# LeonOrou/OPF-Graph-Neural-Solver

Measured on AMD Instinct MI355X. Metric: grids/sec (fwd+bwd) on batched case118, K=4, higher is better.
Workload: dtype f32

## Files before the change

opf-graph-neural-solver_amd/csrc/gns_api.hip:

```cpp
#include <atomic>
#include <cmath>
#include <cstring>
#include <cstdlib>
#include <mutex>
#include <vector>
#include "gns_kernels.h"
#include "gns_gridwg.h"

namespace {
struct GnsTuning {
  int fwd_mapping;
  int gw_pack;
  int fwd_waves;
  int fwd_plane;
  int dw_mfma;
  int train_mapping;
  int bwd_variant;
  int team;
  int bwds_mode;
  int bwds_chunks;
  int bwds_save;
};

bool waves_ok(int& w) { return w > 0 && (w & (w - 1)) == 0 && w * 64 <= GNS_FWD_MAX_THREADS; }
bool chunks_ok(int& c) { return c == 0 || gns_part_index(c) >= 0; }
bool as_flag(int& v) { v = v ? 1 : 0; return true; }
int env_int(const char* e) { return std::atoi(e); }
int env_mapping(const char* e) { return !std::strcmp(e, "lane") ? 1 : (!std::strcmp(e, "lds") ? 2 : 0); }
int env_plane(const char* e) { return e[0] == '0' ? 0 : (e[0] == '1' ? 1 : 2); }
int env_flag(const char* e) { return e[0] == '0' ? 0 : 1; }
struct GnsOption {
  const char* name; int GnsTuning::*member; int lo, hi; bool (*check)(int&); const char* env; int (*parse)(const char*);
  bool accepts(int& v) const { return check ? check(v) : (v >= lo && v <= hi); }
};
const GnsOption g_options[] = {
  {"fwd_mapping",   &GnsTuning::fwd_mapping,   0, 2,            nullptr,   "GNS_FWD_MAPPING",   env_mapping},
  {"train_mapping", &GnsTuning::train_mapping, 0, 2,            nullptr,   "GNS_TRAIN_MAPPING", env_mapping},
  {"bwd_variant",   &GnsTuning::bwd_variant,   1, 4,            nullptr,   "GNS_BWD_VARIANT",   env_int},
  {"gw_pack",       &GnsTuning::gw_pack,       0, 16,           nullptr,   "GNS_GW_PACK",       env_int},
  {"fwd_waves",     &GnsTuning::fwd_waves,     0, 0,            waves_ok,  "GNS_FWD_WAVES",     env_int},
  {"fwd_plane",     &GnsTuning::fwd_plane,     0, 2,            nullptr,   "GNS_FWD_PLANE",     env_plane},
  {"dw_mfma",       &GnsTuning::dw_mfma,       0, 0,            as_flag,   "GNS_DW_MFMA",       env_flag},
  {"team",          &GnsTuning::team,          0, GNS_MAX_TEAM, nullptr,   "GNS_TEAM",          env_int},
  {"bwds_mode",     &GnsTuning::bwds_mode,     0, 2,            nullptr,   "GNS_BWDS_MODE",     env_int},
  {"bwds_chunks",   &GnsTuning::bwds_chunks,   0, 0,            chunks_ok, "GNS_BWDS_CHUNKS",   env_int},
  {"bwds_save",     &GnsTuning::bwds_save,     0, 1,            nullptr,   "GNS_BWDS_SAVE",     env_int},
};
GnsTuning make_tuning() {
  GnsTuning t{0, 0, GNS_FWD_THREADS / 64, 2, 1, 0, 4, 0, 1, 0, 1};
  for (const GnsOption& o : g_options)
    if (const char* e = std::getenv(o.env)) { int v = o.parse(e); if (o.accepts(v)) t.*o.member = v; }
  return t;
}
GnsTuning& tuning() {
  static GnsTuning t = make_tuning();
  return t;
}

struct GnsLast {
  int fwd_kernel, fwd_waves, fwd_plane, team, gw_pack;
  int bwd_kernel, dw_mfma, bwds_mode, bwds_chunks, bwds_R, bwd_gw_pack;
  int bwds_save;
};
GnsLast g_last{-1, -1, -1, -1, -1, -1, -1, -1, -1, -1, -1, -1};
struct GnsLastName { const char* name; int GnsLast::*member; };
const GnsLastName g_last_names[] = {
  {"fwd_kernel", &GnsLast::fwd_kernel}, {"fwd_waves", &GnsLast::fwd_waves}, {"fwd_plane", &GnsLast::fwd_plane}, {"team", &GnsLast::team},
  {"gw_pack", &GnsLast::gw_pack}, {"bwd_kernel", &GnsLast::bwd_kernel}, {"dw_mfma", &GnsLast::dw_mfma}, {"bwds_mode", &GnsLast::bwds_mode},
  {"bwds_chunks", &GnsLast::bwds_chunks}, {"bwds_R", &GnsLast::bwds_R}, {"bwd_gw_pack", &GnsLast::bwd_gw_pack},
  {"bwds_save", &GnsLast::bwds_save},
};
void record_forward(int kernel, int waves, int plane, int team, int pack) {
  g_last.fwd_kernel = kernel; g_last.fwd_waves = waves; g_last.fwd_plane = plane; g_last.team = team; g_last.gw_pack = pack;
}
void record_backward(int kernel, int dw_mfma, int mode, int chunks, int R, int pack, int save = 0) {
  g_last.bwd_kernel = kernel; g_last.dw_mfma = dw_mfma; g_last.bwds_mode = mode; g_last.bwds_chunks = chunks; g_last.bwds_R = R;
  g_last.bwd_gw_pack = pack; g_last.bwds_save = save;
}

constexpr int GNS_MAX_DEVICES = 64;
struct GnsDevice {
  int ncu;
  int gw_ready;
  int split_ready;
  int fwd_ready;
};
const GnsDevice& device() {
  static GnsDevice devs[GNS_MAX_DEVICES];
  static std::atomic<int> done[GNS_MAX_DEVICES];
  static std::mutex mu;
  static const GnsDevice none{0, 0, 0, 0};
  int dev = 0;
// ... 239 lines not shown
int lane_forward(const gns_config* cfg, const GnsFamilies& fam, const GnsFwdLayout& L, char* ws, float* pt, float* pin,
                 const int* topo_dev, const int* group_topo, const int* slot_grid, int64_t Bt, float* v, float* theta,
                 float* total_loss, float* last_loss, int save_state, hipStream_t st) {
  const int N = cfg->n_bus, E = cfg->n_line, K = cfg->K, d = cfg->latent_dim, h = cfg->hidden_dim;
  const GnsTuning& T = tuning();
  int rc;
  GnsFwdArgs A;
  std::memset(&A, 0, sizeof(A));
  A.topo = topo_dev; A.group_topo = group_topo; A.slot_grid = slot_grid; A.pt = pt; A.in = pin;
  A.state = (float*)(ws + L.off_state); A.lam = (float*)(ws + L.off_lam); A.msg = (float*)(ws + L.off_msg);
  A.v_out = v; A.theta_out = theta; A.total_out = total_loss; A.last_out = last_loss;
  fill_forward_families(A, fam);
  fill_loss_weights(A, cfg);
  A.Bt = Bt; A.G = L.groups; A.N = N; A.E = E; A.K = K; A.save = save_state ? 1 : 0;
  A.save_a1 = saves_first_layer(cfg, save_state, group_topo != nullptr) ? 1 : 0;
  const int team0 = lane_team(L.groups * GNS_LANES);
  A.team = team0;
  A.team_ws = (unsigned char*)(ws + L.off_team);
  int waves = T.fwd_waves;
  while (waves * A.team > GNS_MAXP) waves /= 2;
  A.part_idx = gns_part_index(waves * A.team);
  auto pick_planes = [&]() {
    A.plane = (device().fwd_ready && gns_fwd_plane_fits(N, A.team) && T.fwd_plane) ? 1 : 0;
    if (A.plane && gns_fwd_plane2_fits(N, A.team) && T.fwd_plane == 2) A.plane = 2;
  };
  pick_planes();
  if (A.team > 1) {
    const int per_cu = gns_fwd_blocks_per_cu(d, h, cfg->multiple_phi, A, waves * 64);
    if ((long long)per_cu * device().ncu < A.G * A.team) {
      A.team = 1;
      waves = T.fwd_waves;
      A.part_idx = gns_part_index(waves);
      pick_planes();
    }
  }
  if (team0 > 1 && hipMemsetAsync(A.team_ws, 0, (size_t)L.groups * GNS_TEAM_CTR_BYTES, st) != hipSuccess) return GNS_ELAUNCH;
  record_forward(1, waves, A.plane, A.team, -1);
  prof_mark(0, true, st);
  rc = gns_launch_forward(d, h, cfg->multiple_phi, A, waves * 64, st);
  prof_mark(0, false, st);
  return rc;
}

int split_backward(const gns_config* cfg, const GnsFamilies& fam, const GnsFwdLayout& L, const GnsBwdsLayout& S, const char* fw,
                   char* bw, const int* topo_dev, const int* group_topo, const int* slot_grid, const float* params,
                   const void* packed_inputs, int64_t Bt, const float* grad_total, const float* grad_last, const float* grad_v,
                   const float* grad_theta, float* grad_params, hipStream_t st, const IgradOut* ig = nullptr) {
  const int N = cfg->n_bus, E = cfg->n_line, K = cfg->K, d = cfg->latent_dim, h = cfg->hidden_dim;
  int rc;
  GnsBwdsArgs A;
  std::memset(&A, 0, sizeof(A));
  A.topo = topo_dev; A.group_topo = group_topo; A.slot_grid = slot_grid;
  A.pt = (const float*)(fw + L.off_pt); A.pn = (const float*)(fw + L.off_pn);
  A.in = packed_inputs ? (const float*)packed_inputs : (const float*)(fw + L.off_in);
  A.state = (const float*)(fw + L.off_state); A.lam = (const float*)(fw + L.off_lam); A.msg = (const float*)(fw + L.off_msg);
  A.g_total = grad_total; A.g_last = grad_last; A.g_v = grad_v; A.g_theta = grad_theta;
  A.adj = (float*)(bw + S.off_adj); A.slots = (float*)(bw + S.off_slots); A.slab = (float*)(bw + S.off_slab);
  fill_backward_families(A, fam);
  A.Bt = Bt; A.G = S.groups; A.slab_floats = S.slab_floats; A.N = N; A.E = E; A.K = K;
  A.C = S.C; A.part_idx = gns_part_index(S.C); A.R = S.R;
  A.RB = (int)(1 + S.mq); A.RBA = (int)S.adj_rows;
  A.mode = cfg->multiple_phi ? tuning().bwds_mode : 2;
  const size_t lds = gns_bwds_phys_lds(N, &A.use_plane);
  if (ig) {
    A.igrad = ig->buf;
    if (hipMemsetAsync(A.igrad, 0, ig->bytes, st) != hipSuccess) return GNS_ELAUNCH;
  }
  A.save_a1 = saves_first_layer(cfg, ig ? GNS_SAVE_IGRAD : 1, group_topo != nullptr) ? 1 : 0;
  record_backward(4, 1, A.mode, A.C, A.R, -1, A.save_a1);
  prof_mark(1, true, st);
  for (int k = K - 1; k >= 0; --k) {
    A.k = k;
    A.gwk = loss_weight(cfg, k);
    rc = gns_launch_bwds_phys(A, lds, st);
    if (rc != GNS_OK) return rc;
    if (ig) {
      rc = gns_launch_bwds_igrad_phys(A, st);
      if (rc != GNS_OK) return rc;
    }
    rc = gns_launch_bwds_sweep(d, h, cfg->multiple_phi, A, st);
    if (rc != GNS_OK) return rc;
  }
  if (ig && (ig->buses || ig->lines || ig->gens)) {
    rc = gns_launch_bwds_igrad_unpack(A, ig->in_buses, ig->in_lines, ig->in_gens, cfg->n_gen, ig->buses, ig->lines, ig->gens, st);
// ... 442 lines not shown
```

opf-graph-neural-solver_amd/csrc/gns_backward_split.hip:

```cpp
#include "gns_device.h"
#include "gns_kernels.h"
#include "gns_dw.h"
#include "gns_phys_device.h"

typedef int gns_i8v __attribute__((ext_vector_type(8)));
#ifndef GNS_BWDS_ONE_LAYOUT
#define GNS_BWDS_ONE_LAYOUT 0
#endif
#ifndef GNS_BWDS_WPE
#define GNS_BWDS_WPE 2
#endif
#ifndef GNS_BWDS_KEEP_SLOPES
#define GNS_BWDS_KEEP_SLOPES 1
#endif
#if GNS_BWDS_KEEP_SLOPES
#define GNS_SLOPES(sl) sl
#define GNS_SLOPE_OF(sl, layer, act, u) sl[layer][u]
#else
#define GNS_SLOPES(sl) nullptr
#define GNS_SLOPE_OF(sl, layer, act, u) dlrelu2(act[u])
#endif
#ifndef GNS_BWDS_FRESH_INPUTS
#define GNS_BWDS_FRESH_INPUTS 1
#endif
// ... 5 lines not shown
#endif
#ifndef GNS_BWDS_AH_M
#define GNS_BWDS_AH_M 5
#endif
#ifndef GNS_BWDS_AH_M0
#define GNS_BWDS_AH_M0 5
#endif
#ifndef GNS_BWDS_AH_T0
#define GNS_BWDS_AH_T0 4
#endif
#ifndef GNS_BWDS_LASTK_FOLD
#define GNS_BWDS_LASTK_FOLD 0
#endif
#define GNS_BWDS_PHYS_THREADS (GNS_BWDS_PHYS_WAVES * 64)

__global__ void __launch_bounds__(GNS_BWDS_PHYS_THREADS) gns_bwds_phys_kernel(GnsBwdsArgs A) {
  extern __shared__ __attribute__((aligned(16))) float lds[];
  constexpr int W = GNS_BWDS_PHYS_WAVES;
  const int lane = threadIdx.x & 63;
  const int wave = __builtin_amdgcn_readfirstlane(threadIdx.x >> 6);
  const int N = A.N, E = A.E, K = A.K, k = A.k;
  cip topo = (cip)A.topo;
  const long long g = blockIdx.x;
  long long b = g * GNS_LANES + lane;
  bool live = b < A.Bt;
  if (A.group_topo) {
    const int s = A.slot_grid[g * GNS_LANES + lane];
    b = s;
    live = s >= 0 && s < A.Bt;
    if (!gns_group_topo(A.topo, A.group_topo, g, N, E, topo)) return;
// ... 7 lines not shown
  const int e0 = epart[wave], e1 = epart[wave + 1];
  const bool use_plane = A.use_plane != 0, plane_dp = A.use_plane == 2;
  float* const red = lds;
  float* const pl_v = lds + W * GNS_LANES;
  float* const pl_th = pl_v + (use_plane ? N * GNS_LANES : 0);
  float* const pl_dp = pl_th + (plane_dp ? N * GNS_LANES : 0);
  const long long R = gns_in_rows(N, E);
  const float* IN = A.in;
  const long long in_base = g * R, row_ein = in_base + 3LL * N, row_eout = row_ein + 3LL * E, row_grid = row_eout + E;
  const float gt = (live && A.g_total) ? A.g_total[b] : 0.f;
  const float gl = (live && A.g_last) ? A.g_last[b] : 0.f;
  const int RB = A.RB, RBA = A.RBA;
  auto state_row = [&](int slot, int n) { return (((long long)slot * A.G + g) * N + n) * RB; };
  auto adj_row = [&](int n) { return (g * N + n) * RBA; };
  auto slot_ptr = [&](int j, int p) { return A.slots + ((g * 6 + j) * E + p) * GNS_LANES + lane; };
  const f4 gsum = *row_ptr(IN, row_grid, lane);
  const float invN = 1.0f / (float)N;
  const bool last = k == K - 1;
  const int mode = A.mode;
  const bool x2_live = mode == 2 || k + 1 < K - 1;
  const float cdp = 2.f * (gt * A.gwk + (last ? gl : 0.f)) * invN;
  const f2 lamv = reinterpret_cast<const f2*>(A.lam)[((long long)k * A.G + g) * GNS_LANES + lane];
  const int bits = (int)lamv.y;
  const bool low1 = bits & 1, low2 = bits & 2;

  float lb = 0.f;
  constexpr int PB = 4;
  for (int nb = n0; nb < n1; nb += PB) {
    f4 s1[PB], a0[PB], x0[PB], x1[PB], x2[PB], b1[PB];
#pragma unroll
// ... 58 lines not shown
        L.thc = pl_th[ic * GNS_LANES + lane]; L.thd = pl_th[id * GNS_LANES + lane];
        if (plane_dp) { L.Fb = pl_dp[t * GNS_LANES + lane]; L.Tb = pl_dp[s * GNS_LANES + lane]; }
        else { L.Fb = row_ptr(A.adj, adj_row(t), lane)->z; L.Tb = row_ptr(A.adj, adj_row(s), lane)->z; }
      } else {
        const f4 ss = *row_ptr(A.state, state_row(k + 1, s), lane), st = *row_ptr(A.state, state_row(k + 1, t), lane);
        L.vs = ss.x; L.ths = ss.y; L.vt = st.x; L.tht = st.y;
        L.tha = row_ptr(A.state, state_row(k + 1, ia), lane)->y; L.thb = row_ptr(A.state, state_row(k + 1, ib), lane)->y;
        L.thc = row_ptr(A.state, state_row(k + 1, ic), lane)->y; L.thd = row_ptr(A.state, state_row(k + 1, id), lane)->y;
        L.Fb = row_ptr(A.adj, adj_row(t), lane)->z;
        L.Tb = row_ptr(A.adj, adj_row(s), lane)->z;
      }
    };
    auto edge_adjoint = [&](int p, const EdgeIn& L) {
      const LineTrig T = line_trig<false>(L.ths, L.tht, L.tha, L.thb, L.thc, L.thd, L.e1v.w, L.o0.z);
      const LineAdj R = line_state_adjoint(T, L.vs, L.vt, L.e1v.y, L.e1v.z, L.o0.x, L.o0.y, L.Fb, L.Tb, pgbar);
      if (!L.gs) *slot_ptr(0, p) = R.dvs;
      if (!L.gt) *slot_ptr(1, p) = R.dvt;
      *slot_ptr(2, p) = R.dths;
      *slot_ptr(4, p) = R.dbar; *slot_ptr(5, p) = R.dbar2;
    };
    for (int p = e0; p < e1; p += 2) {
      EdgeIn L0, L1;
      edge_load(p, L0);
      edge_load(min(p + 1, e1 - 1), L1);
      edge_adjoint(p, L0);
      if (p + 1 < e1) edge_adjoint(p + 1, L1);
    }
  }
  __syncthreads();

  for (int n = n0; n < n1; ++n) {
    const long long ar = adj_row(n);
    const f4 a0 = *row_ptr(A.adj, ar, lane);
    float vbar = a0.x, thbar = a0.y;
    const float dpb = a0.z;
    const int p0 = in_ptr[n], p1 = in_ptr[n + 1], q0 = out_ptr[n], q1 = out_ptr[n + 1], i0 = incd_ptr[n], i1 = incd_ptr[n + 1];
    const bool gen = is_gen[n] != 0;
    {
      float ai[4], bi[4], ao[4], bo[4], ci[8];
#pragma unroll
      for (int j = 0; j < 4; ++j) { const int pp = min(p0 + j, max(p1 - 1, p0)); ai[j] = gen ? 0.f : *slot_ptr(1, min(pp, E - 1)); bi[j] = -*slot_ptr(2, min(pp, E - 1)); }
#pragma unroll
      for (int j = 0; j < 4; ++j) { const int p = q2p[min(min(q0 + j, max(q1 - 1, q0)), E - 1)]; ao[j] = gen ? 0.f : *slot_ptr(0, p); bo[j] = *slot_ptr(2, p); }
#pragma unroll
      for (int j = 0; j < 8; ++j) {
        const int code = incd[min(min(i0 + j, max(i1 - 1, i0)), 4 * E - 1)];
        const float val = *slot_ptr((code & 2) ? 5 : 4, code >> 2);
        ci[j] = (code & 1) ? -val : val;
      }
#pragma unroll
      for (int j = 0; j < 4; ++j) if (p0 + j < p1) { vbar += ai[j]; thbar += bi[j]; }
#pragma unroll
      for (int j = 0; j < 4; ++j) if (q0 + j < q1) { vbar += ao[j]; thbar += bo[j]; }
#pragma unroll
      for (int j = 0; j < 8; ++j) if (i0 + j < i1) thbar += ci[j];
    }
    for (int p = p0 + 4; p < p1; p += 4) {
      float a[4], bb[4];
#pragma unroll
      for (int j = 0; j < 4; ++j) { const int pp = min(p + j, p1 - 1); a[j] = gen ? 0.f : *slot_ptr(1, pp); bb[j] = -*slot_ptr(2, pp); }
#pragma unroll
      for (int j = 0; j < 4; ++j) if (p + j < p1) { vbar += a[j]; thbar += bb[j]; }
    }
    for (int q = q0 + 4; q < q1; q += 4) {
      float a[4], bb[4];
#pragma unroll
      for (int j = 0; j < 4; ++j) { const int p = q2p[min(q + j, q1 - 1)]; a[j] = gen ? 0.f : *slot_ptr(0, p); bb[j] = *slot_ptr(2, p); }
#pragma unroll
      for (int j = 0; j < 4; ++j) if (q + j < q1) { vbar += a[j]; thbar += bb[j]; }
    }
    for (int i = i0 + 8; i < i1; i += 8) {
      float a[8];
#pragma unroll
      for (int j = 0; j < 8; ++j) {
        const int code = incd[min(i + j, i1 - 1)];
        const float val = *slot_ptr((code & 2) ? 5 : 4, code >> 2);
        a[j] = (code & 1) ? -val : val;
      }
#pragma unroll
      for (int j = 0; j < 8; ++j) if (i + j < i1) thbar += a[j];
    }
    vbar += (pgbar - dpb) * a0.w;
    *row_ptr(A.adj, ar, lane) = f4{vbar, thbar, dpb, 0.f};
  }
}

template <int D, int H, bool MULTI>
struct BwdsShape {
  using C = GnsDims<D, H, MULTI>;
  static constexpr int LIN = C::LF_IN, XL = (LIN + 1) / 2, PIN = C::PHI_IN, SOFF = 2 + D / 2;
  static constexpr int NB1 = (2 * XL + 15) / 16, NDM = (D + 15) / 16;
// ... 692 lines not shown
int gns_launch_bwds_igrad_unpack(const GnsBwdsArgs& A, const float* buses, const float* lines, const float* gens, int Gn,
                                 float* grad_buses, float* grad_lines, float* grad_gens, hipStream_t st) {
  hipLaunchKernelGGL(gns_bwds_igrad_unpack_kernel, dim3((unsigned)A.G, (unsigned)(A.N + A.E)), dim3(64), 0, st, A, buses, lines, gens, Gn,
                     grad_buses, grad_lines, grad_gens);
  return hipGetLastError() == hipSuccess ? GNS_OK : GNS_ELAUNCH;
}

int gns_bwds_supported(int d, int h, int multi) {
  (void)multi;
#define GNS_CASE(DD, HH) if (d == DD && h == HH) return 1;
  GNS_FOR_EACH_DIMS(GNS_CASE)
#undef GNS_CASE
  return 0;
}

size_t gns_bwds_phys_lds(int N, int* use_plane) {
  const size_t red = (size_t)GNS_BWDS_PHYS_WAVES * GNS_LANES * 4;
  const size_t plane = (size_t)N * GNS_LANES * 4;
  const int level = red + 3 * plane <= (size_t)160 * 1024 ? 2 : (red + 2 * plane <= (size_t)160 * 1024 ? 1 : 0);
  if (use_plane) *use_plane = level;
  return red + (level == 2 ? 3 : (level == 1 ? 2 : 0)) * plane;
}

int gns_launch_bwds_phys(const GnsBwdsArgs& A, size_t lds, hipStream_t st) {
  hipLaunchKernelGGL(gns_bwds_phys_kernel, dim3((unsigned)A.G), dim3(GNS_BWDS_PHYS_THREADS), lds, st, A);
  return hipGetLastError() == hipSuccess ? GNS_OK : GNS_ELAUNCH;
}

int gns_launch_bwds_sweep(int d, int h, int multi, const GnsBwdsArgs& A, hipStream_t st) {
  const long long GB = (A.G + A.R - 1) / A.R;
  const unsigned blocks = (unsigned)(GB * A.C);
  const bool fold_m = GNS_BWDS_LASTK_FOLD && A.k == A.K - 1 && !A.group_topo && !A.igrad;
#define GNS_SWEEP1(DD, HH, MM, FAMS, GR, IG) do { if (A.k == 0) hipLaunchKernelGGL((gns_bwds_sweep_kernel<DD, HH, MM, FAMS, true, GR, IG>), dim3(blocks), dim3(64), 0, st, A); \
                                                 else hipLaunchKernelGGL((gns_bwds_sweep_kernel<DD, HH, MM, FAMS, false, GR, IG>), dim3(blocks), dim3(64), 0, st, A); } while (0)
#define GNS_SWEEP(DD, HH, MM, FAMS) do { if (A.group_topo) GNS_SWEEP1(DD, HH, MM, FAMS, true, false); \
                                         else if (A.igrad) GNS_SWEEP1(DD, HH, MM, FAMS, false, true); \
                                         else GNS_SWEEP1(DD, HH, MM, FAMS, false, false); } while (0)
  if (A.save_a1) {
    if (d != 20 || h != 10 || !multi || A.mode != 1 || A.group_topo || A.igrad) return GNS_EINVAL;
#define GNS_SAVED(FAMS) do { if (A.k == 0) hipLaunchKernelGGL((gns_bwds_sweep_kernel<20, 10, true, FAMS, true, false, false, true>), dim3(blocks), dim3(64), 0, st, A); \
// ... 7 lines not shown
  if (d == DD && h == HH) {                                                                                                 \
    if (!multi) { if (A.mode != 2) return GNS_EINVAL; GNS_SWEEP(DD, HH, false, 7); }                                        \
    else if (A.mode == 2) GNS_SWEEP(DD, HH, true, 7);                                                                       \
    else if (A.mode == 1) { if (!fold_m) GNS_SWEEP(DD, HH, true, 4); GNS_SWEEP(DD, HH, true, 3); }                          \
    else { if (!fold_m) GNS_SWEEP(DD, HH, true, 4); GNS_SWEEP(DD, HH, true, 1); GNS_SWEEP(DD, HH, true, 2); }               \
    return hipGetLastError() == hipSuccess ? GNS_OK : GNS_ELAUNCH;                                                          \
  }
  GNS_FOR_EACH_DIMS(GNS_CASE)
#undef GNS_CASE
#undef GNS_SWEEP
#undef GNS_SWEEP1
  return GNS_EUNSUPPORTED;
}

int gns_bwds_init_device() {
  return hipFuncSetAttribute((const void*)gns_bwds_phys_kernel, hipFuncAttributeMaxDynamicSharedMemorySize, 160 * 1024) == hipSuccess
             ? GNS_OK : GNS_ELAUNCH;
}
```

opf-graph-neural-solver_amd/csrc/gns_forward.hip:

```cpp
#include "gns_device.h"
#ifndef GNS_FWD_GEN_SKIP
#define GNS_FWD_GEN_SKIP 1
#endif
#include "gns_kernels.h"

__global__ void gns_pack_params_kernel(const float* __restrict__ flat, float* __restrict__ pt, float* __restrict__ pn,
                                       GnsFamilies fam, int K, int D, int H) {
  const int blk = blockIdx.x;
  const int f = blk / K, k = blk % K;
  const bool is_phi = f < fam.nphi;
  const int Dr = fam.dr, Hr = fam.hr;
  const int INr = fam.in[f], OUTr = fam.out[f];
  const int OUT = fam.outk[f], OUTP = OUT + (OUT & 1);
  const float* src = flat + fam.flat_off[f] + (int64_t)k * fam.flat_sz[f];
  const int sW1 = 0, sb1 = INr * Hr, sW2 = sb1 + Hr, sb2 = sW2 + Hr * Hr, sW4 = sb2 + Hr, sb4 = sW4 + OUTr * Hr;
  auto W2r = [&](int j, int i) -> float { return (j < Hr && i < Hr) ? src[sW2 + j * Hr + i] : 0.f; };
  auto b1r = [&](int j) -> float { return j < Hr ? src[sb1 + j] : 0.f; };
  auto b2r = [&](int j) -> float { return j < Hr ? src[sb2 + j] : 0.f; };
  float* t = pt + fam.t_off[f] + (int64_t)k * fam.t_sz[f];
  float* n = pn + fam.n_off[f] + (int64_t)k * fam.n_sz[f];
  if (is_phi) {
    const int IN = D + 5, INP = IN + (IN & 1);
    auto W1r = [&](int j, int i) -> float {
      if (j >= Hr) return 0.f;
// ... 105 lines not shown
    }
    const float v0 = (vg == 0.f) ? 1.f : vg;
    put(3LL * n, bq);
    put(3LL * n + 1, f4{pmin, pset, pmax, bq.z});
    put(3LL * n + 2, f4{__fsub_rn(__fsub_rn(pg, bq.x), __fmul_rn(bq.z, __fmul_rn(v0, v0))),
                        __fadd_rn(__fsub_rn(qg, bq.y), __fmul_rn(bq.w, __fmul_rn(v0, v0))), v0, 0.f});
  } else if (c < cb + ci) {
    const int p = (c - cb) * W + wave;
    if (p >= E) return;
    const int e = topo[topo[TH_IN_EID] + p], s = topo[topo[TH_IN_SRC] + p];
    const f4 ea = ld4(li + e * 7 + 2);
    const float she = li[e * 7 + 6];
    const f4 sa = ld4(li + s * 7 + 2);
    const float shs = li[s * 7 + 6];
    put(3LL * N + 3LL * p, ea);
    put(3LL * N + 3LL * p + 1, f4{she, yof(sa.x, sa.y), sa.w, shs});
    put(3LL * N + 3LL * p + 2, f4{sa.z, 0.f, 0.f, 0.f});
  } else if (c < cb + ci + co) {
    const int q0 = ((c - cb - ci) * W + wave) * 4;
    f4 ta[4];
    float sh[4];
#pragma unroll
    for (int i = 0; i < 4; ++i) {
      const int t = topo[topo[TH_OUT_DST] + min(q0 + i, E - 1)];
      ta[i] = ld4(li + t * 7 + 2);
      sh[i] = li[t * 7 + 6];
    }
#pragma unroll
    for (int i = 0; i < 4; ++i)
      if (q0 + i < E) put(3LL * N + 3LL * E + q0 + i, f4{yof(ta[i].x, ta[i].y), ta[i].w, sh[i], ta[i].z});
  } else {
    if (wave != 0) return;
    float sPd = 0.f, sset = 0.f, smin = 0.f, smax = 0.f;
#pragma unroll 8
    for (int n = 0; n < N; ++n) sPd += bu[n * 6 + 2];
#pragma unroll 4
    for (int q = 0; q < Gn; ++q) { const f2 pm = ld2(ge + q * 7 + 1); smax += pm.x; smin += pm.y; sset += ge[q * 7 + 3]; }
    put(3LL * N + 4LL * E, f4{sPd, sset, smin, smax});
  }
}

#ifndef GNS_FWD_SKIP_LAST_M
#define GNS_FWD_SKIP_LAST_M 1
#endif
#ifndef GNS_FWD_ROW_STORES
#define GNS_FWD_ROW_STORES 0
#endif
template <int D, int H, bool MULTI, bool GROUPED, bool SAVE_A1 = false>
__global__ void __launch_bounds__(GNS_FWD_MAX_THREADS) gns_forward_kernel(GnsFwdArgs A) {
  using C = GnsDims<D, H, MULTI>;
  constexpr int MQ = C::MQ, RB = C::RB;
  constexpr bool save_a1 = SAVE_A1;
  const int lane = threadIdx.x & 63;
  const int wave = __builtin_amdgcn_readfirstlane(threadIdx.x >> 6);
  const int nwaves = blockDim.x >> 6;
  const int tsize = A.team;
  long long g = blockIdx.x;
  int member = 0;
  if (tsize > 1) {
    if ((A.G & 7) == 0) { g = (long long)(blockIdx.x / (8 * tsize)) * 8 + (blockIdx.x & 7); member = (blockIdx.x >> 3) % tsize; }
    else { g = blockIdx.x / tsize; member = blockIdx.x % tsize; }
  }
  const int cw = member * nwaves + wave, tw = tsize * nwaves;
  const int N = A.N, E = A.E, K = A.K;
  cip topo = (cip)A.topo;
  long long b = g * GNS_LANES + lane;
  bool live = b < A.Bt;
// ... 194 lines not shown
    auto vth = [&](int n) {
      if (use_plane) return plane[n * GNS_LANES + lane];
      const f4 r = *row_ptr(A.state, state_row(ws, n), lane);
      return f2{r.x, r.y};
    };
    float joule = 0.f, v2gs = 0.f;
    for (int n = q0w; n < q1w; ++n) {
      const long long wr = state_row(ws, n);
      const f2 sn = vth(n);
      const float vn = sn.x, thn = sn.y;
      const f4 b0 = *row_ptr(IN, in_base + 3LL * n, lane);
      float sum_pf = 0.f, sum_qf = 0.f, sum_pt = 0.f, sum_qt = 0.f, agg = 0.f;
      const int p0 = in_ptr[n], p1 = in_ptr[n + 1];
      for (int p = p0; p < p1; ++p) {
        const int s = in_src[p], ia = in_a[p], ib = in_b[p];
        const f4 e1 = *row_ptr(IN, row_ein + 3LL * p + 1, lane), e2 = *row_ptr(IN, row_ein + 3LL * p + 2, lane);
        const f2 ss = vth(s);
        const float tha = vth(ia).y, thb = vth(ib).y;
        const float vs = ss.x, ths = ss.y, vt = vn, tht = thn;
        const float ys = e1.y, taus = e1.z, shs = e1.w, bs = e2.x;
        const float dl = tha - thb;
        const float angA = ths - tht - dl - shs, angB = tht - ths - dl + shs;
        float sA, cA, sD, cD;
        sincosf(angA, &sA, &cA);
        sincosf(dl, &sD, &cD);
        const float sB = sinf(angB);
        const float base = vs * vt * ys / taus;
        const float msg = fabsf(base * (sA + sB) + (vs / (taus * taus)) * ys * sD + (vt * vt) * ys * sD);
        agg += msg;
        const float vst = vs / taus, vst2 = vst * vst;
        sum_pf += base * sA + vst2 * ys * sD;
        sum_qf += -base * cA + vst2 * (ys * cD - bs / 2.f);
      }
      const int q0 = out_ptr[n], q1 = out_ptr[n + 1];
      for (int q = q0; q < q1; ++q) {
// ... 28 lines not shown
    red_sum(k & 1, jsum, vsum);
    const float p_global = (gsum.x + vsum) + jsum;
    float lam;
    const bool low1 = p_global < gsum.y;
    if (low1) lam = (p_global - gsum.z) / (2.f * (gsum.y - gsum.z));
    else lam = (p_global - 2.f * gsum.y + gsum.w) / (2.f * (gsum.w - gsum.y));
    const bool low2 = lam < 0.5f;
    if (A.save && cw == 0)
      reinterpret_cast<f2*>(A.lam)[((long long)k * A.G + g) * GNS_LANES + lane] = f2{lam, (low1 ? 1.f : 0.f) + (low2 ? 2.f : 0.f)};
    float sq = 0.f;
    for (int nb = q0w; nb < q1w; nb += 4) {
      f4 b1[4], sn[4];
#pragma unroll
      for (int j = 0; j < 4; ++j) {
        const int n = min(nb + j, q1w - 1);
        b1[j] = *row_ptr(IN, in_base + 3LL * n + 1, lane);
        if (use_plane2) {
          const f2 vt_ = plane[n * GNS_LANES + lane], pq_ = plane2[n * GNS_LANES + lane];
          sn[j] = f4{vt_.x, vt_.y, pq_.x, pq_.y};
        } else {
          sn[j] = *row_ptr(A.state, state_row(ws, n), lane);
        }
      }
#pragma unroll
      for (int j = 0; j < 4; ++j) {
        if (nb + j < q1w) {
          const float pg = low2 ? b1[j].x + 2.f * (b1[j].y - b1[j].x) * lam
                                : 2.f * b1[j].y - b1[j].z + 2.f * (b1[j].z - b1[j].y) * lam;
          sn[j].z = pg + sn[j].z;
          *row_ptr(A.state, state_row(ws, nb + j), lane) = sn[j];
          sq += sn[j].z * sn[j].z + sn[j].w * sn[j].w;
// ... 25 lines not shown
    red_sum(0, t, l);
    if (team_failed) t = l = __builtin_nanf("");
    A.total_out[b] = t;
    A.last_out[b] = l;
  }
  if (tsize > 1 && team_failed && threadIdx.x == 0)
    __hip_atomic_store(reinterpret_cast<unsigned*>(A.team_ws) + GNS_TEAM_STATUS_WORD, 1u, __ATOMIC_RELAXED, __HIP_MEMORY_SCOPE_AGENT);
}

static size_t fwd_dyn_lds(const GnsFwdArgs& A) {
  return (A.plane ? (size_t)A.N * GNS_LANES * sizeof(f2) : 0) * (A.plane == 2 ? 2 : 1) + (A.team == 1 ? (size_t)GNS_FWD_RED_BYTES : 0);
}

template <int D, int H, bool MULTI>
static int launch_forward_t(const GnsFwdArgs& A, int threads, hipStream_t st) {
  if (A.group_topo) hipLaunchKernelGGL((gns_forward_kernel<D, H, MULTI, true>), dim3((unsigned)(A.G * A.team)), dim3(threads), fwd_dyn_lds(A), st, A);
  else if (A.save_a1) {
    if constexpr (D == 20 && H == 10 && MULTI) hipLaunchKernelGGL((gns_forward_kernel<D, H, MULTI, false, true>), dim3((unsigned)(A.G * A.team)), dim3(threads), fwd_dyn_lds(A), st, A);
    else return GNS_EINVAL;
  }
  else hipLaunchKernelGGL((gns_forward_kernel<D, H, MULTI, false>), dim3((unsigned)(A.G * A.team)), dim3(threads), fwd_dyn_lds(A), st, A);
  return hipGetLastError() == hipSuccess ? GNS_OK : GNS_ELAUNCH;
}

int gns_fwd_init_device() {
  int rc = GNS_OK;
#define GNS_CASE(DD, HH)                                                                                                              \
  if (hipFuncSetAttribute(reinterpret_cast<const void*>(&gns_forward_kernel<DD, HH, true, false>), hipFuncAttributeMaxDynamicSharedMemorySize, GNS_FWD_DYN_LDS_MAX) != hipSuccess) rc = GNS_ELAUNCH;   \
  if (hipFuncSetAttribute(reinterpret_cast<const void*>(&gns_forward_kernel<DD, HH, false, false>), hipFuncAttributeMaxDynamicSharedMemorySize, GNS_FWD_DYN_LDS_MAX) != hipSuccess) rc = GNS_ELAUNCH;   \
  if (hipFuncSetAttribute(reinterpret_cast<const void*>(&gns_forward_kernel<DD, HH, true, true>), hipFuncAttributeMaxDynamicSharedMemorySize, GNS_FWD_DYN_LDS_MAX) != hipSuccess) rc = GNS_ELAUNCH;   \
  if (hipFuncSetAttribute(reinterpret_cast<const void*>(&gns_forward_kernel<DD, HH, false, true>), hipFuncAttributeMaxDynamicSharedMemorySize, GNS_FWD_DYN_LDS_MAX) != hipSuccess) rc = GNS_ELAUNCH;
  GNS_FOR_EACH_DIMS(GNS_CASE)
#undef GNS_CASE
  if (hipFuncSetAttribute(reinterpret_cast<const void*>(&gns_forward_kernel<20, 10, true, false, true>), hipFuncAttributeMaxDynamicSharedMemorySize, GNS_FWD_DYN_LDS_MAX) != hipSuccess) rc = GNS_ELAUNCH;
  if (rc != GNS_OK) (void)hipGetLastError();
  return rc;
}

int gns_fwd_blocks_per_cu(int d, int h, int multi, const GnsFwdArgs& A, int threads) {
  int nb = 0;
#define GNS_CASE(DD, HH)                                                                                                              \
  if (d == DD && h == HH) {                                                                                                           \
    const size_t lds = fwd_dyn_lds(A);                                                                                                \
    const hipError_t e = A.group_topo                                                                                                 \
        ? (multi ? hipOccupancyMaxActiveBlocksPerMultiprocessor(&nb, gns_forward_kernel<DD, HH, true, true>, threads, lds)              \
                 : hipOccupancyMaxActiveBlocksPerMultiprocessor(&nb, gns_forward_kernel<DD, HH, false, true>, threads, lds))            \
        : (multi ? hipOccupancyMaxActiveBlocksPerMultiprocessor(&nb, gns_forward_kernel<DD, HH, true, false>, threads, lds)             \
                 : hipOccupancyMaxActiveBlocksPerMultiprocessor(&nb, gns_forward_kernel<DD, HH, false, false>, threads, lds));          \
    if (e != hipSuccess) { (void)hipGetLastError(); return 0; }                                                                       \
// ... 32 lines not shown
```

opf-graph-neural-solver_amd/csrc/gns_kernels.h:

```cpp
#pragma once
#include <hip/hip_runtime.h>
#include "../../include/gns_hip.h"
#include "gns_common.h"

#define GNS_FWD_THREADS 1024
#define GNS_FWD_MAX_THREADS 1024
#define GNS_BWD_THREADS 512
#define GNS_MAX_K 64
#define GNS_FWD_RED_BYTES (2 * GNS_MAXW * GNS_LANES * 2 * 4)
#define GNS_FWD_DYN_LDS_MAX (160 * 1024 - 64)
static inline int gns_fwd_plane_fits(int N, int team) {
  return (size_t)N * GNS_LANES * 8 + (team == 1 ? GNS_FWD_RED_BYTES : 0) <= (size_t)GNS_FWD_DYN_LDS_MAX;
}
static inline int gns_fwd_plane2_fits(int N, int team) {
  return team == 1 && 2 * (size_t)N * GNS_LANES * 8 + GNS_FWD_RED_BYTES <= (size_t)GNS_FWD_DYN_LDS_MAX;
}

#define GNS_FOR_EACH_DIMS(X) X(20, 14) X(20, 10) X(10, 10)
#define GNS_FOR_EACH_DIMS_PERSISTENT(X) X(20, 10) X(10, 10)
#define GNS_FOR_EACH_DIMS_GWB(X) X(20, 10) X(10, 10)

template <int D, int H, bool MULTI>
struct GnsDims {
  static constexpr int NPHI = MULTI ? 3 : 1;
// ... 13 lines not shown
  const float* in;
  float* state;
  float* lam;
  float* msg;
  float* v_out; float* theta_out; float* total_out; float* last_out;
  long long t_off[6], t_sz[6];
  float gw[GNS_MAX_K];
  long long Bt, G;
  int N, E, K, save, part_idx;
  int plane;
  int team;
  unsigned char* team_ws;
  const int* group_topo;
  const int* slot_grid;
  int save_a1;
};

struct GnsBwdArgs {
  const int* topo;
  const float* pt; const float* pn;
  const float* in;
  const float* state;
  const float* lam;
  const float* msg;
  const float* g_total; const float* g_last; const float* g_v; const float* g_theta;
  float* adj;
  float* slots;
  float* slab;
  long long t_off[6], t_sz[6], n_off[6], n_sz[6], g_off[6], g_sz[6];
  float gw[GNS_MAX_K];
// ... 21 lines not shown
  const float* in; const float* state; const float* lam; const float* msg;
  const float* g_total; const float* g_last; const float* g_v; const float* g_theta;
  float* adj; float* slots; float* slab;
  long long t_off[6], t_sz[6], n_off[6], n_sz[6], g_off[6], g_sz[6];
  long long Bt, G, slab_floats;
  float gwk;
  int N, E, K, k;
  int C, part_idx, R;
  int RB, RBA;
  int use_plane;
  int mode;
  const int* group_topo;
  const int* slot_grid;
  float* igrad;
  int save_a1;
};
int gns_bwds_supported(int d, int h, int multi);
size_t gns_bwds_phys_lds(int N, int* use_plane);
int gns_launch_bwds_phys(const GnsBwdsArgs& A, size_t lds, hipStream_t st);
int gns_launch_bwds_sweep(int d, int h, int multi, const GnsBwdsArgs& A, hipStream_t st);
int gns_launch_bwds_igrad_phys(const GnsBwdsArgs& A, hipStream_t st);
int gns_launch_bwds_igrad_unpack(const GnsBwdsArgs& A, const float* buses, const float* lines, const float* gens, int Gn,
                                 float* grad_buses, float* grad_lines, float* grad_gens, hipStream_t st);
int gns_bwds_init_device();
```

Before: 6.301 million.

## Keep backward edge-slot adjoints in LDS and trim forward edge-row loads

Result: no change. 6.294 million, median of 2 (-0.1%).

```diff
diff --git a/opf-graph-neural-solver_amd/csrc/gns_api.hip b/opf-graph-neural-solver_amd/csrc/gns_api.hip
--- a/opf-graph-neural-solver_amd/csrc/gns_api.hip
+++ b/opf-graph-neural-solver_amd/csrc/gns_api.hip
@@ -20,6 +20,8 @@
   int bwds_mode;
   int bwds_chunks;
   int bwds_save;
+  int fwd_rows;
+  int phys_slots;
 };
 
 bool waves_ok(int& w) { return w > 0 && (w & (w - 1)) == 0 && w * 64 <= GNS_FWD_MAX_THREADS; }
@@ -45,9 +47,11 @@
   {"bwds_mode",     &GnsTuning::bwds_mode,     0, 2,            nullptr,   "GNS_BWDS_MODE",     env_int},
   {"bwds_chunks",   &GnsTuning::bwds_chunks,   0, 0,            chunks_ok, "GNS_BWDS_CHUNKS",   env_int},
   {"bwds_save",     &GnsTuning::bwds_save,     0, 1,            nullptr,   "GNS_BWDS_SAVE",     env_int},
+  {"fwd_rows",      &GnsTuning::fwd_rows,      0, 1,            nullptr,   "GNS_FWD_ROWS",      env_int},
+  {"phys_slots",    &GnsTuning::phys_slots,    0, 1,            nullptr,   "GNS_PHYS_SLOTS",    env_int},
 };
 GnsTuning make_tuning() {
-  GnsTuning t{0, 0, GNS_FWD_THREADS / 64, 2, 1, 0, 4, 0, 1, 0, 1};
+  GnsTuning t{0, 0, GNS_FWD_THREADS / 64, 2, 1, 0, 4, 0, 1, 0, 1, 1, 1};
   for (const GnsOption& o : g_options)
     if (const char* e = std::getenv(o.env)) { int v = o.parse(e); if (o.accepts(v)) t.*o.member = v; }
   return t;
@@ -61,21 +65,24 @@
   int fwd_kernel, fwd_waves, fwd_plane, team, gw_pack;
   int bwd_kernel, dw_mfma, bwds_mode, bwds_chunks, bwds_R, bwd_gw_pack;
   int bwds_save;
-};
-GnsLast g_last{-1, -1, -1, -1, -1, -1, -1, -1, -1, -1, -1, -1};
+  int fwd_rows;
+  int phys_slots;
+};
+GnsLast g_last{-1, -1, -1, -1, -1, -1, -1, -1, -1, -1, -1, -1, -1, -1};
 struct GnsLastName { const char* name; int GnsLast::*member; };
 const GnsLastName g_last_names[] = {
   {"fwd_kernel", &GnsLast::fwd_kernel}, {"fwd_waves", &GnsLast::fwd_waves}, {"fwd_plane", &GnsLast::fwd_plane}, {"team", &GnsLast::team},
   {"gw_pack", &GnsLast::gw_pack}, {"bwd_kernel", &GnsLast::bwd_kernel}, {"dw_mfma", &GnsLast::dw_mfma}, {"bwds_mode", &GnsLast::bwds_mode},
   {"bwds_chunks", &GnsLast::bwds_chunks}, {"bwds_R", &GnsLast::bwds_R}, {"bwd_gw_pack", &GnsLast::bwd_gw_pack},
-  {"bwds_save", &GnsLast::bwds_save},
-};
-void record_forward(int kernel, int waves, int plane, int team, int pack) {
+  {"bwds_save", &GnsLast::bwds_save}, {"fwd_rows", &GnsLast::fwd_rows}, {"phys_slots", &GnsLast::phys_slots},
+};
+void record_forward(int kernel, int waves, int plane, int team, int pack, int rows = -1) {
   g_last.fwd_kernel = kernel; g_last.fwd_waves = waves; g_last.fwd_plane = plane; g_last.team = team; g_last.gw_pack = pack;
-}
-void record_backward(int kernel, int dw_mfma, int mode, int chunks, int R, int pack, int save = 0) {
+  g_last.fwd_rows = rows;
+}
+void record_backward(int kernel, int dw_mfma, int mode, int chunks, int R, int pack, int save = 0, int slot_planes = -1) {
   g_last.bwd_kernel = kernel; g_last.dw_mfma = dw_mfma; g_last.bwds_mode = mode; g_last.bwds_chunks = chunks; g_last.bwds_R = R;
-  g_last.bwd_gw_pack = pack; g_last.bwds_save = save;
+  g_last.bwd_gw_pack = pack; g_last.bwds_save = save; g_last.phys_slots = slot_planes;
 }
 
 constexpr int GNS_MAX_DEVICES = 64;
@@ -345,6 +352,7 @@
   fill_loss_weights(A, cfg);
   A.Bt = Bt; A.G = L.groups; A.N = N; A.E = E; A.K = K; A.save = save_state ? 1 : 0;
   A.save_a1 = saves_first_layer(cfg, save_state, group_topo != nullptr) ? 1 : 0;
+  A.fwd_rows = T.fwd_rows;
   const int team0 = lane_team(L.groups * GNS_LANES);
   A.team = team0;
   A.team_ws = (unsigned char*)(ws + L.off_team);
@@ -366,7 +374,7 @@
     }
   }
   if (team0 > 1 && hipMemsetAsync(A.team_ws, 0, (size_t)L.groups * GNS_TEAM_CTR_BYTES, st) != hipSuccess) return GNS_ELAUNCH;
-  record_forward(1, waves, A.plane, A.team, -1);
+  record_forward(1, waves, A.plane, A.team, -1, A.fwd_rows);
   prof_mark(0, true, st);
   rc = gns_launch_forward(d, h, cfg->multiple_phi, A, waves * 64, st);
   prof_mark(0, false, st);
@@ -392,13 +400,13 @@
   A.C = S.C; A.part_idx = gns_part_index(S.C); A.R = S.R;
   A.RB = (int)(1 + S.mq); A.RBA = (int)S.adj_rows;
   A.mode = cfg->multiple_phi ? tuning().bwds_mode : 2;
-  const size_t lds = gns_bwds_phys_lds(N, &A.use_plane);
+  const size_t lds = gns_bwds_phys_lds(N, E, tuning().phys_slots ? GNS_BWDS_SLOT_PLANES : 0, &A.use_plane, &A.slot_planes);
   if (ig) {
     A.igrad = ig->buf;
     if (hipMemsetAsync(A.igrad, 0, ig->bytes, st) != hipSuccess) return GNS_ELAUNCH;
   }
   A.save_a1 = saves_first_layer(cfg, ig ? GNS_SAVE_IGRAD : 1, group_topo != nullptr) ? 1 : 0;
-  record_backward(4, 1, A.mode, A.C, A.R, -1, A.save_a1);
+  record_backward(4, 1, A.mode, A.C, A.R, -1, A.save_a1, A.slot_planes);
   prof_mark(1, true, st);
   for (int k = K - 1; k >= 0; --k) {
     A.k = k;
diff --git a/opf-graph-neural-solver_amd/csrc/gns_backward_split.hip b/opf-graph-neural-solver_amd/csrc/gns_backward_split.hip
--- a/opf-graph-neural-solver_amd/csrc/gns_backward_split.hip
+++ b/opf-graph-neural-solver_amd/csrc/gns_backward_split.hip
@@ -43,6 +43,7 @@
 #endif
 #define GNS_BWDS_PHYS_THREADS (GNS_BWDS_PHYS_WAVES * 64)
 
+template <int NSL>
 __global__ void __launch_bounds__(GNS_BWDS_PHYS_THREADS) gns_bwds_phys_kernel(GnsBwdsArgs A) {
   extern __shared__ __attribute__((aligned(16))) float lds[];
   constexpr int W = GNS_BWDS_PHYS_WAVES;
@@ -80,6 +81,18 @@
   auto state_row = [&](int slot, int n) { return (((long long)slot * A.G + g) * N + n) * RB; };
   auto adj_row = [&](int n) { return (g * N + n) * RBA; };
   auto slot_ptr = [&](int j, int p) { return A.slots + ((g * 6 + j) * E + p) * GNS_LANES + lane; };
+  constexpr int nsl = NSL;
+  float* const pl_slot = pl_dp + (plane_dp ? N * GNS_LANES : 0);
+  auto slot_rank = [](int j) { return j == 2 ? 0 : (j == 4 ? 1 : (j == 5 ? 2 : (j == 0 ? 3 : 4))); };
+  auto slot_st = [&](int j, int p, float x) {
+    const int r = slot_rank(j);
+    if (r < nsl) pl_slot[(r * E + p) * GNS_LANES + lane] = x;
+    else *slot_ptr(j, p) = x;
+  };
+  auto slot_ld = [&](int j, int p) -> float {
+    const int r = slot_rank(j);
+    return r < nsl ? pl_slot[(r * E + p) * GNS_LANES + lane] : *slot_ptr(j, p);
+  };
   const f4 gsum = *row_ptr(IN, row_grid, lane);
   const float invN = 1.0f / (float)N;
   const bool last = k == K - 1;
@@ -168,10 +181,10 @@
     auto edge_adjoint = [&](int p, const EdgeIn& L) {
       const LineTrig T = line_trig<false>(L.ths, L.tht, L.tha, L.thb, L.thc, L.thd, L.e1v.w, L.o0.z);
       const LineAdj R = line_state_adjoint(T, L.vs, L.vt, L.e1v.y, L.e1v.z, L.o0.x, L.o0.y, L.Fb, L.Tb, pgbar);
-      if (!L.gs) *slot_ptr(0, p) = R.dvs;
-      if (!L.gt) *slot_ptr(1, p) = R.dvt;
-      *slot_ptr(2, p) = R.dths;
-      *slot_ptr(4, p) = R.dbar; *slot_ptr(5, p) = R.dbar2;
+      if (!L.gs) slot_st(0, p, R.dvs);
+      if (!L.gt) slot_st(1, p, R.dvt);
+      slot_st(2, p, R.dths);
+      slot_st(4, p, R.dbar); slot_st(5, p, R.dbar2);
     };
     for (int p = e0; p < e1; p += 2) {
       EdgeIn L0, L1;
@@ -193,13 +206,13 @@
     {
       float ai[4], bi[4], ao[4], bo[4], ci[8];
 #pragma unroll
-      for (int j = 0; j < 4; ++j) { const int pp = min(p0 + j, max(p1 - 1, p0)); ai[j] = gen ? 0.f : *slot_ptr(1, min(pp, E - 1)); bi[j] = -*slot_ptr(2, min(pp, E - 1)); }
-#pragma unroll
-      for (int j = 0; j < 4; ++j) { const int p = q2p[min(min(q0 + j, max(q1 - 1, q0)), E - 1)]; ao[j] = gen ? 0.f : *slot_ptr(0, p); bo[j] = *slot_ptr(2, p); }
+      for (int j = 0; j < 4; ++j) { const int pp = min(p0 + j, max(p1 - 1, p0)); ai[j] = gen ? 0.f : slot_ld(1, min(pp, E - 1)); bi[j] = -slot_ld(2, min(pp, E - 1)); }
+#pragma unroll
+      for (int j = 0; j < 4; ++j) { const int p = q2p[min(min(q0 + j, max(q1 - 1, q0)), E - 1)]; ao[j] = gen ? 0.f : slot_ld(0, p); bo[j] = slot_ld(2, p); }
 #pragma unroll
       for (int j = 0; j < 8; ++j) {
         const int code = incd[min(min(i0 + j, max(i1 - 1, i0)), 4 * E - 1)];
-        const float val = *slot_ptr((code & 2) ? 5 : 4, code >> 2);
+        const float val = slot_ld((code & 2) ? 5 : 4, code >> 2);
         ci[j] = (code & 1) ? -val : val;
       }
 #pragma unroll
@@ -212,14 +225,14 @@
     for (int p = p0 + 4; p < p1; p += 4) {
       float a[4], bb[4];
 #pragma unroll
-      for (int j = 0; j < 4; ++j) { const int pp = min(p + j, p1 - 1); a[j] = gen ? 0.f : *slot_ptr(1, pp); bb[j] = -*slot_ptr(2, pp); }
+      for (int j = 0; j < 4; ++j) { const int pp = min(p + j, p1 - 1); a[j] = gen ? 0.f : slot_ld(1, pp); bb[j] = -slot_ld(2, pp); }
 #pragma unroll
       for (int j = 0; j < 4; ++j) if (p + j < p1) { vbar += a[j]; thbar += bb[j]; }
     }
     for (int q = q0 + 4; q < q1; q += 4) {
       float a[4], bb[4];
 #pragma unroll
-      for (int j = 0; j < 4; ++j) { const int p = q2p[min(q + j, q1 - 1)]; a[j] = gen ? 0.f : *slot_ptr(0, p); bb[j] = *slot_ptr(2, p); }
+      for (int j = 0; j < 4; ++j) { const int p = q2p[min(q + j, q1 - 1)]; a[j] = gen ? 0.f : slot_ld(0, p); bb[j] = slot_ld(2, p); }
 #pragma unroll
       for (int j = 0; j < 4; ++j) if (q + j < q1) { vbar += a[j]; thbar += bb[j]; }
     }
@@ -228,7 +241,7 @@
 #pragma unroll
       for (int j = 0; j < 8; ++j) {
         const int code = incd[min(i + j, i1 - 1)];
-        const float val = *slot_ptr((code & 2) ? 5 : 4, code >> 2);
+        const float val = slot_ld((code & 2) ? 5 : 4, code >> 2);
         a[j] = (code & 1) ? -val : val;
       }
 #pragma unroll
@@ -951,16 +964,31 @@
   return 0;
 }
 
+static constexpr size_t GNS_BWDS_PHYS_LDS_CAP = (size_t)160 * 1024;
 size_t gns_bwds_phys_lds(int N, int* use_plane) {
   const size_t red = (size_t)GNS_BWDS_PHYS_WAVES * GNS_LANES * 4;
   const size_t plane = (size_t)N * GNS_LANES * 4;
-  const int level = red + 3 * plane <= (size_t)160 * 1024 ? 2 : (red + 2 * plane <= (size_t)160 * 1024 ? 1 : 0);
+  const int level = red + 3 * plane <= GNS_BWDS_PHYS_LDS_CAP ? 2 : (red + 2 * plane <= GNS_BWDS_PHYS_LDS_CAP ? 1 : 0);
   if (use_plane) *use_plane = level;
   return red + (level == 2 ? 3 : (level == 1 ? 2 : 0)) * plane;
 }
+size_t gns_bwds_phys_lds(int N, int E, int max_slot_planes, int* use_plane, int* slot_planes) {
+  const size_t cap = GNS_BWDS_PHYS_LDS_CAP;
+  const size_t buses = gns_bwds_phys_lds(N, use_plane);
+  const size_t slot = (size_t)E * GNS_LANES * 4;
+  int ns = 0;
+  while (ns < max_slot_planes && ns < GNS_BWDS_SLOT_PLANES && buses + (size_t)(ns + 1) * slot <= cap) ++ns;
+  if (slot_planes) *slot_planes = ns;
+  return buses + (size_t)ns * slot;
+}
 
 int gns_launch_bwds_phys(const GnsBwdsArgs& A, size_t lds, hipStream_t st) {
-  hipLaunchKernelGGL(gns_bwds_phys_kernel, dim3((unsigned)A.G), dim3(GNS_BWDS_PHYS_THREADS), lds, st, A);
+  switch (A.slot_planes) {
+#define GNS_CASE(NS) case NS: hipLaunchKernelGGL(gns_bwds_phys_kernel<NS>, dim3((unsigned)A.G), dim3(GNS_BWDS_PHYS_THREADS), lds, st, A); break;
+  GNS_CASE(0) GNS_CASE(1) GNS_CASE(2) GNS_CASE(3) GNS_CASE(4) GNS_CASE(5)
+#undef GNS_CASE
+  default: return GNS_EINVAL;
+  }
   return hipGetLastError() == hipSuccess ? GNS_OK : GNS_ELAUNCH;
 }
 
@@ -998,6 +1026,11 @@
 }
 
 int gns_bwds_init_device() {
-  return hipFuncSetAttribute((const void*)gns_bwds_phys_kernel, hipFuncAttributeMaxDynamicSharedMemorySize, 160 * 1024) == hipSuccess
-             ? GNS_OK : GNS_ELAUNCH;
-}
+  int rc = GNS_OK;
+#define GNS_CASE(NS) if (hipFuncSetAttribute((const void*)gns_bwds_phys_kernel<NS>, hipFuncAttributeMaxDynamicSharedMemorySize, 160 * 1024) != hipSuccess) rc = GNS_ELAUNCH;
+  GNS_CASE(0) GNS_CASE(1) GNS_CASE(2) GNS_CASE(3) GNS_CASE(4) GNS_CASE(5)
+#undef GNS_CASE
+  static_assert(GNS_BWDS_SLOT_PLANES == 5, "one instantiation of gns_bwds_phys_kernel per plane count");
+  if (rc != GNS_OK) (void)hipGetLastError();
+  return rc;
+}
diff --git a/opf-graph-neural-solver_amd/csrc/gns_forward.hip b/opf-graph-neural-solver_amd/csrc/gns_forward.hip
--- a/opf-graph-neural-solver_amd/csrc/gns_forward.hip
+++ b/opf-graph-neural-solver_amd/csrc/gns_forward.hip
@@ -143,8 +143,9 @@
     const f4 sa = ld4(li + s * 7 + 2);
     const float shs = li[s * 7 + 6];
     put(3LL * N + 3LL * p, ea);
-    put(3LL * N + 3LL * p + 1, f4{she, yof(sa.x, sa.y), sa.w, shs});
-    put(3LL * N + 3LL * p + 2, f4{sa.z, 0.f, 0.f, 0.f});
+    const float ys = yof(sa.x, sa.y);
+    put(3LL * N + 3LL * p + 1, f4{she, ys, sa.w, shs});
+    put(3LL * N + 3LL * p + 2, f4{sa.z, ys, sa.w, shs});
   } else if (c < cb + ci + co) {
     const int q0 = ((c - cb - ci) * W + wave) * 4;
     f4 ta[4];
@@ -175,11 +176,12 @@
 #ifndef GNS_FWD_ROW_STORES
 #define GNS_FWD_ROW_STORES 0
 #endif
-template <int D, int H, bool MULTI, bool GROUPED, bool SAVE_A1 = false>
+template <int D, int H, bool MULTI, bool GROUPED, bool SAVE_A1 = false, bool ROWS = true>
 __global__ void __launch_bounds__(GNS_FWD_MAX_THREADS) gns_forward_kernel(GnsFwdArgs A) {
   using C = GnsDims<D, H, MULTI>;
   constexpr int MQ = C::MQ, RB = C::RB;
   constexpr bool save_a1 = SAVE_A1;
+  constexpr bool fwd_rows = ROWS;
   const int lane = threadIdx.x & 63;
   const int wave = __builtin_amdgcn_readfirstlane(threadIdx.x >> 6);
   const int nwaves = blockDim.x >> 6;
@@ -404,11 +406,17 @@
       const int p0 = in_ptr[n], p1 = in_ptr[n + 1];
       for (int p = p0; p < p1; ++p) {
         const int s = in_src[p], ia = in_a[p], ib = in_b[p];
-        const f4 e1 = *row_ptr(IN, row_ein + 3LL * p + 1, lane), e2 = *row_ptr(IN, row_ein + 3LL * p + 2, lane);
+        float ys, taus, shs, bs;
+        if constexpr (fwd_rows) {
+          const f4 e2 = *row_ptr(IN, row_ein + 3LL * p + 2, lane);
+          bs = e2.x; ys = e2.y; taus = e2.z; shs = e2.w;
+        } else {
+          const f4 e1 = *row_ptr(IN, row_ein + 3LL * p + 1, lane), e2 = *row_ptr(IN, row_ein + 3LL * p + 2, lane);
+          ys = e1.y; taus = e1.z; shs = e1.w; bs = e2.x;
+        }
         const f2 ss = vth(s);
         const float tha = vth(ia).y, thb = vth(ib).y;
         const float vs = ss.x, ths = ss.y, vt = vn, tht = thn;
-        const float ys = e1.y, taus = e1.z, shs = e1.w, bs = e2.x;
         const float dl = tha - thb;
         const float angA = ths - tht - dl - shs, angB = tht - ths - dl + shs;
         float sA, cA, sD, cD;
@@ -467,7 +475,8 @@
 #pragma unroll
       for (int j = 0; j < 4; ++j) {
         const int n = min(nb + j, q1w - 1);
-        b1[j] = *row_ptr(IN, in_base + 3LL * n + 1, lane);
+        if (!fwd_rows || is_gen[n] != 0) b1[j] = *row_ptr(IN, in_base + 3LL * n + 1, lane);
+        else b1[j] = f4{0.f, 0.f, 0.f, 0.f};
         if (use_plane2) {
           const f2 vt_ = plane[n * GNS_LANES + lane], pq_ = plane2[n * GNS_LANES + lane];
           sn[j] = f4{vt_.x, vt_.y, pq_.x, pq_.y};
@@ -523,25 +532,31 @@
 
 template <int D, int H, bool MULTI>
 static int launch_forward_t(const GnsFwdArgs& A, int threads, hipStream_t st) {
-  if (A.group_topo) hipLaunchKernelGGL((gns_forward_kernel<D, H, MULTI, true>), dim3((unsigned)(A.G * A.team)), dim3(threads), fwd_dyn_lds(A), st, A);
+#define GNS_FWD_GO(GR, SV) do { if (A.fwd_rows) hipLaunchKernelGGL((gns_forward_kernel<D, H, MULTI, GR, SV, true>), dim3((unsigned)(A.G * A.team)), dim3(threads), fwd_dyn_lds(A), st, A); \
+                                else hipLaunchKernelGGL((gns_forward_kernel<D, H, MULTI, GR, SV, false>), dim3((unsigned)(A.G * A.team)), dim3(threads), fwd_dyn_lds(A), st, A); } while (0)
+  if (A.group_topo) GNS_FWD_GO(true, false);
   else if (A.save_a1) {
-    if constexpr (D == 20 && H == 10 && MULTI) hipLaunchKernelGGL((gns_forward_kernel<D, H, MULTI, false, true>), dim3((unsigned)(A.G * A.team)), dim3(threads), fwd_dyn_lds(A), st, A);
+    if constexpr (D == 20 && H == 10 && MULTI) GNS_FWD_GO(false, true);
     else return GNS_EINVAL;
   }
-  else hipLaunchKernelGGL((gns_forward_kernel<D, H, MULTI, false>), dim3((unsigned)(A.G * A.team)), dim3(threads), fwd_dyn_lds(A), st, A);
+  else GNS_FWD_GO(false, false);
+#undef GNS_FWD_GO
   return hipGetLastError() == hipSuccess ? GNS_OK : GNS_ELAUNCH;
 }
 
 int gns_fwd_init_device() {
   int rc = GNS_OK;
-#define GNS_CASE(DD, HH)                                                                                                              \
-  if (hipFuncSetAttribute(reinterpret_cast<const void*>(&gns_forward_kernel<DD, HH, true, false>), hipFuncAttributeMaxDynamicSharedMemorySize, GNS_FWD_DYN_LDS_MAX) != hipSuccess) rc = GNS_ELAUNCH;   \
-  if (hipFuncSetAttribute(reinterpret_cast<const void*>(&gns_forward_kernel<DD, HH, false, false>), hipFuncAttributeMaxDynamicSharedMemorySize, GNS_FWD_DYN_LDS_MAX) != hipSuccess) rc = GNS_ELAUNCH;   \
-  if (hipFuncSetAttribute(reinterpret_cast<const void*>(&gns_forward_kernel<DD, HH, true, true>), hipFuncAttributeMaxDynamicSharedMemorySize, GNS_FWD_DYN_LDS_MAX) != hipSuccess) rc = GNS_ELAUNCH;   \
-  if (hipFuncSetAttribute(reinterpret_cast<const void*>(&gns_forward_kernel<DD, HH, false, true>), hipFuncAttributeMaxDynamicSharedMemorySize, GNS_FWD_DYN_LDS_MAX) != hipSuccess) rc = GNS_ELAUNCH;
+  auto opt_in = [&](const void* kernel) {
+    if (hipFuncSetAttribute(kernel, hipFuncAttributeMaxDynamicSharedMemorySize, GNS_FWD_DYN_LDS_MAX) != hipSuccess) rc = GNS_ELAUNCH;
+  };
+#define GNS_BOTH(DD, HH, MM, GR, SV)                                                                     \
+  opt_in(reinterpret_cast<const void*>(&gns_forward_kernel<DD, HH, MM, GR, SV, true>));                   \
+  opt_in(reinterpret_cast<const void*>(&gns_forward_kernel<DD, HH, MM, GR, SV, false>));
+#define GNS_CASE(DD, HH) GNS_BOTH(DD, HH, true, false, false) GNS_BOTH(DD, HH, false, false, false) GNS_BOTH(DD, HH, true, true, false) GNS_BOTH(DD, HH, false, true, false)
   GNS_FOR_EACH_DIMS(GNS_CASE)
 #undef GNS_CASE
-  if (hipFuncSetAttribute(reinterpret_cast<const void*>(&gns_forward_kernel<20, 10, true, false, true>), hipFuncAttributeMaxDynamicSharedMemorySize, GNS_FWD_DYN_LDS_MAX) != hipSuccess) rc = GNS_ELAUNCH;
+  GNS_BOTH(20, 10, true, false, true)
+#undef GNS_BOTH
   if (rc != GNS_OK) (void)hipGetLastError();
   return rc;
 }
diff --git a/opf-graph-neural-solver_amd/csrc/gns_kernels.h b/opf-graph-neural-solver_amd/csrc/gns_kernels.h
--- a/opf-graph-neural-solver_amd/csrc/gns_kernels.h
+++ b/opf-graph-neural-solver_amd/csrc/gns_kernels.h
@@ -51,6 +51,7 @@
   const int* group_topo;
   const int* slot_grid;
   int save_a1;
+  int fwd_rows;
 };
 
 struct GnsBwdArgs {
@@ -102,9 +103,12 @@
   const int* slot_grid;
   float* igrad;
   int save_a1;
+  int slot_planes;
 };
+#define GNS_BWDS_SLOT_PLANES 5
 int gns_bwds_supported(int d, int h, int multi);
 size_t gns_bwds_phys_lds(int N, int* use_plane);
+size_t gns_bwds_phys_lds(int N, int E, int max_slot_planes, int* use_plane, int* slot_planes);
 int gns_launch_bwds_phys(const GnsBwdsArgs& A, size_t lds, hipStream_t st);
 int gns_launch_bwds_sweep(int d, int h, int multi, const GnsBwdsArgs& A, hipStream_t st);
 int gns_launch_bwds_igrad_phys(const GnsBwdsArgs& A, hipStream_t st);
```
